# huangnengCSU/NanoSNP

Hardware: AMD Instinct MI355X
Metric: candidate SNP sites/sec (pileup encode + model fwd), 30x windows (higher is better)
Workload: dtype f32; 1 GPU; BASELINE configs[1]: pileup encode + PileupModel fwd, 1M synthetic 30x windows (G2) resident in HBM, batch=4096; batch=4096, windows_resident_per_gpu=1048576, streams=32, precision=fp32, parallelism=site-sharded x1, rooted gather of calls, world_size_observed=1, gather=torch

## Files before the change

### nanosnp_amd/csrc/nsnp_lstm_cell.hpp

```cpp
#pragma once

namespace nsnp_cell {

constexpr float LOG2E = 1.4426950408889634f;

static inline float lstm_gate_scale(int R) { return (R & 3) == 2 ? -2.0f * LOG2E : -LOG2E; }

__device__ __forceinline__ float cap64(float z) { return __builtin_amdgcn_fmed3f(z, -3.0e38f, 64.0f); }

__device__ __forceinline__ float lstm_cell(float zi, float zf, float zg, float zo, float c_prev, float& c_new)
{
    const float ei = __builtin_amdgcn_exp2f(zi);
    const float ef = __builtin_amdgcn_exp2f(zf);
    const float eo = __builtin_amdgcn_exp2f(zo);
    const float eg = __builtin_amdgcn_exp2f(cap64(zg));
    constexpr float K = -2.0f * LOG2E;
    const float tg = 1.0f + eg;
    const float ig = __builtin_fmaf(-K, eg, K) * __builtin_amdgcn_rcpf(__builtin_fmaf(ei, tg, tg));
    const float fg = __builtin_amdgcn_rcpf(1.0f + ef);
    const float cn = __builtin_fmaf(fg, c_prev, ig);
    const float ec = __builtin_amdgcn_exp2f(cap64(cn));
    c_new = cn;
    const float tc = 1.0f + ec;
    return (1.0f - ec) * __builtin_amdgcn_rcpf(__builtin_fmaf(eo, tc, tc));
}

struct CellSlices { float ei[4], ef[4], eo[4], eg[4], t[4], d[4], m[4], fg[4]; };
constexpr int CELL_SLICES = 80;

template <int I, typename Z4>
__device__ __forceinline__ void lstm_cell_slice(CellSlices& w, const Z4 (&z)[4], float (&c)[4], Z4& h)
{
    static_assert(I >= 0 && I < CELL_SLICES, "slice index");
    constexpr int st = I >> 2, u = I & 3;
    constexpr float K = -2.0f * LOG2E;
    if constexpr (st == 0) w.ei[u] = __builtin_amdgcn_exp2f(z[u][0]);
    else if constexpr (st == 1) w.ef[u] = __builtin_amdgcn_exp2f(z[u][1]);
    else if constexpr (st == 2) w.eo[u] = __builtin_amdgcn_exp2f(z[u][3]);
    else if constexpr (st == 3) w.t[u] = cap64(z[u][2]);
    else if constexpr (st == 4) w.eg[u] = __builtin_amdgcn_exp2f(w.t[u]);
    else if constexpr (st == 5) w.t[u] = 1.0f + w.eg[u];
    else if constexpr (st == 6) w.d[u] = __builtin_fmaf(w.ei[u], w.t[u], w.t[u]);
    else if constexpr (st == 7) w.d[u] = __builtin_amdgcn_rcpf(w.d[u]);
    else if constexpr (st == 8) w.m[u] = __builtin_fmaf(-K, w.eg[u], K);
    else if constexpr (st == 9) w.m[u] = w.m[u] * w.d[u];
    else if constexpr (st == 10) w.fg[u] = 1.0f + w.ef[u];
    else if constexpr (st == 11) w.fg[u] = __builtin_amdgcn_rcpf(w.fg[u]);
    else if constexpr (st == 12) c[u] = __builtin_fmaf(w.fg[u], c[u], w.m[u]);
    else if constexpr (st == 13) w.t[u] = cap64(c[u]);
    else if constexpr (st == 14) w.eg[u] = __builtin_amdgcn_exp2f(w.t[u]);
    else if constexpr (st == 15) w.t[u] = 1.0f + w.eg[u];
    else if constexpr (st == 16) w.d[u] = __builtin_fmaf(w.eo[u], w.t[u], w.t[u]);
    else if constexpr (st == 17) w.d[u] = __builtin_amdgcn_rcpf(w.d[u]);
    else if constexpr (st == 18) w.m[u] = 1.0f - w.eg[u];
    else h[u] = w.m[u] * w.d[u];
    if constexpr (st == 0) asm volatile("" : "+v"(w.ei[u]));
    else if constexpr (st == 1) asm volatile("" : "+v"(w.ef[u]));
    else if constexpr (st == 2) asm volatile("" : "+v"(w.eo[u]));
    else if constexpr (st == 4 || st == 14) asm volatile("" : "+v"(w.eg[u]));
    else if constexpr (st == 3 || st == 5 || st == 13 || st == 15) asm volatile("" : "+v"(w.t[u]));
    else if constexpr (st == 6 || st == 7 || st == 16 || st == 17) asm volatile("" : "+v"(w.d[u]));
    else if constexpr (st == 8 || st == 9 || st == 18) asm volatile("" : "+v"(w.m[u]));
    else if constexpr (st == 10 || st == 11) asm volatile("" : "+v"(w.fg[u]));
    else if constexpr (st == 12) asm volatile("" : "+v"(c[u]));
    else { float v = h[u]; asm volatile("" : "+v"(v)); h[u] = v; }
}

}
```

### nanosnp_amd/csrc/pileup_forward.hip

```cpp
#include "nsnp_common.hpp"
#include "nsnp_lstm_cell.hpp"
#include "nsnp_devclock.hpp"
#include "nsnp_bf16.hpp"
#include <type_traits>

namespace {

constexpr float LOG2E = 1.4426950408889634f;

__device__ __forceinline__ f32x4 mfma4(float a, float b, f32x4 c)
{
    return __builtin_amdgcn_mfma_f32_16x16x4f32(a, b, c, 0, 0, 0);
}
__device__ __forceinline__ float sigmoid_f(float x)
{
    return __builtin_amdgcn_rcpf(1.0f + __builtin_amdgcn_exp2f(-LOG2E * x));
}
__device__ __forceinline__ float tanh_f(float x)
{
    return __builtin_fmaf(-2.0f, __builtin_amdgcn_rcpf(1.0f + __builtin_amdgcn_exp2f((2.0f * LOG2E) * x)), 1.0f);
}

__device__ __forceinline__ float lstm_cell(float zi, float zf, float zg, float zo, float& c)
{
// ... 369 lines not shown
            Frag fr[2];
            f32x4 acc[2][4];
            load_b(0, fr[0]);
            gemm(fr[0], acc[0]);
#pragma unroll
            for (int sg = 0; sg < NSG; ++sg) {
                __builtin_amdgcn_sched_barrier(0);
                if (sg + 1 < NSG) load_b(sg + 1, fr[(sg + 1) & 1]);
                __builtin_amdgcn_sched_barrier(0);
                if (sg + 1 < NSG) gemm(fr[(sg + 1) & 1], acc[(sg + 1) & 1]);
                cell(sg, acc[sg & 1]);
                if (sg + 1 < NSG) {
#pragma unroll
                    for (int i = 0; i < 84; ++i) {
                        __builtin_amdgcn_sched_group_barrier(0x008, 1, 0);
                        __builtin_amdgcn_sched_group_barrier(0x400, 1, 0);
                        __builtin_amdgcn_sched_group_barrier(0x002, 1, 0);
                    }
                }
            }
            __builtin_amdgcn_sched_barrier(0);
        } else {
#pragma unroll
        for (int sg = 0; sg < NSG; ++sg) {
            const float* hr = &hx[cur ^ 1][16 * sg + n][4 * q];
            f32x4 hb0, hb1;
            if (s > 0) { hb0 = *reinterpret_cast<const f32x4*>(hr); hb1 = *reinterpret_cast<const f32x4*>(hr + 16); }
            const float* xr = &xx[cur][(16 * sg + n) * RS_XSROW];
            const f32x4 xb = *reinterpret_cast<const f32x4*>(xr + 4 * q);
            const float xl = xr[16 + q];
            f32x4 acc[4];
#pragma unroll
            for (int u = 0; u < 4; ++u) acc[u] = f32x4{0.f, 0.f, 0.f, 0.f};
            if (WXL) {
#pragma unroll
                for (int u = 0; u < 4; ++u) {
                    Wih[u] = *reinterpret_cast<const f32x4*>(&wxl[((wave * 4 + u) * 64 + lane) * 4]);
                    Wl[u] = wxl[4 * 4 * 64 * 4 + (wave * 4 + u) * 64 + lane];
                }
            }
#pragma unroll
            for (int e = 0; e < 4; ++e)
#pragma unroll
                for (int u = 0; u < 4; ++u) acc[u] = mfma4(Wih[u][e], xb[e], acc[u]);
#pragma unroll
            for (int u = 0; u < 4; ++u) acc[u] = mfma4(Wl[u], xl, acc[u]);
            if (s > 0) {
#define RS_KBLOCK(J, HB)                                                                               \
                _Pragma("unroll") for (int e = 0; e < 4; ++e)                                          \
                    _Pragma("unroll") for (int u = 0; u < 4; ++u) acc[u] = mfma4(Whh[u][J][e], HB[e], acc[u]);
                __builtin_amdgcn_sched_barrier(0);
                RS_KBLOCK(0, hb0)
                __builtin_amdgcn_sched_barrier(0);
                hb0 = *reinterpret_cast<const f32x4*>(hr + 32);
                RS_KBLOCK(1, hb1)
                __builtin_amdgcn_sched_barrier(0);
                hb1 = *reinterpret_cast<const f32x4*>(hr + 48);
                RS_KBLOCK(2, hb0)
                __builtin_amdgcn_sched_barrier(0);
                RS_KBLOCK(3, hb1)
#undef RS_KBLOCK
            }
            f32x4 hn;
#pragma unroll
            for (int u = 0; u < 4; ++u) {
                hn[u] = lstm_cell(acc[u][0], acc[u][1], acc[u][2], acc[u][3], c[sg][u]);
            }
            *reinterpret_cast<f32x4*>(&hx[cur][16 * sg + n][16 * wave + 4 * q]) = hn;
        }
        }
        if (s + 1 < PW) {
            stage_x(cur ^ 1);
            if (s + 2 < PW) load_x(dir ? t - 2 : t + 2);
        }
        lds_barrier();
    }
    flush_h((PW - 1) & 1, dir ? 0 : PW - 1);
    NSNP_DEVCLK_STOP(0)
}

constexpr int RX_PLANE = 4 * 16 * 8;
typedef float f32x2 __attribute__((ext_vector_type(2)));

__global__ __launch_bounds__(256, 3) void k_pileup_l0_rsx(
    const int32_t* __restrict__ x, const int64_t* __restrict__ center_idx, int64_t N,
    const float* __restrict__ whh0, const float* __restrict__ whh1,
    const __bf16* __restrict__ wx0, const __bf16* __restrict__ wx1,
    float* __restrict__ H0)
{
    __shared__ __attribute__((aligned(16))) float hx[2][16][RS_XROW];
    __shared__ __attribute__((aligned(16))) __bf16 xx[2][3][RX_PLANE];
    __shared__ __attribute__((aligned(16))) int xlvl[2][4];
    __shared__ int64_t xofs[9 * 16];
    const int dir = blockIdx.y;
    const int tid = threadIdx.x, lane = tid & 63, wave = __builtin_amdgcn_readfirstlane(tid >> 6);
    const int n = lane & 15, q = lane >> 4;
    NSNP_DEVCLK_START
    const int64_t base_site = (int64_t)blockIdx.x * 16;
    const int nrows = (int)min((int64_t)16, N - base_site);

    f32x4 Whh[4][4];
    b8 Wx[4][3];
    {
        const f32x4* __restrict__ ghh = reinterpret_cast<const f32x4*>(dir ? whh1 : whh0);
        const b8* __restrict__ gx = reinterpret_cast<const b8*>(dir ? wx1 : wx0);
#pragma unroll
        for (int u = 0; u < 4; ++u) {
#pragma unroll
            for (int j = 0; j < 4; ++j) Whh[u][j] = ghh[((4 * wave + u) * 4 + j) * 64 + lane];
#pragma unroll
            for (int p = 0; p < 3; ++p) Wx[u][p] = gx[((4 * wave + u) * 3 + p) * 64 + lane];
        }
    }

    const bool xon = tid < 9 * 16;
    const int xrow = min(wave < 2 ? lane >> 2 : n, nrows - 1);
    const int piece = wave < 2 ? 4 * wave + (lane & 3) : 8;
    const int xdst = wave < 2 ? 128 * wave + 2 * lane : 256 + 8 * n;
    const int32_t* const xwg = x + base_site * (PW * PC);
    unsigned xoff = (unsigned)(xrow * (PW * PC) + 2 * piece) * 4u;
    if (center_idx && xon) xofs[tid] = (center_idx[base_site + xrow] - PCENTER) * PC + 2 * piece;
    int2 xi = int2{0, 0};
    auto load_x = [&](int t) {
        if (!xon) return;
        if (center_idx) xi = *reinterpret_cast<const int2*>(x + xofs[tid] + t * PC);
        else {
            asm volatile("" : "+v"(xoff));
            xi = *reinterpret_cast<const int2*>(reinterpret_cast<const char*>(xwg + t * PC) + xoff);
        }
    };
    auto stage_x_split = [&](b2* d, int* lv) {
        __bf16 a0, a1, a2, c0, c1, c2;
        split3((float)xi.x, a0, a1, a2); split3((float)xi.y, c0, c1, c2);
        d[0] = b2{a0, c0}; d[RX_PLANE / 2] = b2{a1, c1}; d[RX_PLANE] = b2{a2, c2};
        const bool nz1 = (float)a1 != 0.f || (float)c1 != 0.f, nz2 = (float)a2 != 0.f || (float)c2 != 0.f;
        const int lvl = __ballot(nz2) != 0ull ? 2 : (__ballot(nz1) != 0ull ? 1 : 0);
        if (lane == 0) *lv = lvl;
    };
    auto stage_x = [&](int buf) {
        if (!xon) return;
        b2* const d = reinterpret_cast<b2*>(&xx[buf][0][xdst]);
        const bool big = (unsigned)xi.x + 256u > 512u || (unsigned)xi.y + 256u > 512u;
        if (__builtin_expect(__ballot(big) == 0ull, 1)) {
            d[0] = __builtin_convertvector(f32x2{(float)xi.x, (float)xi.y}, b2);
            d[RX_PLANE / 2] = b2{0, 0};
            d[RX_PLANE] = b2{0, 0};
            if (lane == 0) xlvl[buf][wave] = 0;
        } else {
            stage_x_split(d, &xlvl[buf][wave]);
        }
    };
    for (int i = tid; i < 2 * 3 * RX_PLANE / 8; i += 256) reinterpret_cast<b8*>(&xx[0][0][0])[i] = b8{0, 0, 0, 0, 0, 0, 0, 0};
    if (tid < 8) xlvl[tid >> 2][tid & 3] = 0;
    __syncthreads();
    if (tid < 32) xx[tid >> 4][0][2 * 128 + (tid & 15) * 8 + 2] = (__bf16)1.0f;
    load_x(dir ? PW - 1 : 0);
    stage_x(0);
    if (PW > 1) load_x(dir ? PW - 2 : 1);
    __syncthreads();

    float c[4];
#pragma unroll
    for (int u = 0; u < 4; ++u) c[u] = 0.f;

    float* const h0wg = H0 + (base_site * PW * 2 + dir) * 64;
    const int frow = tid >> 4, fcid = tid & 15;
    unsigned foff = (unsigned)(frow * (PW * 128) + 4 * fcid) * 4u;
    const float* const fl = &hx[0][frow][16 * (fcid & 3) + 4 * (fcid >> 2)];
    const bool fon = frow < nrows;
    auto flush_h = [&](int buf, int t) {
        asm volatile("" : "+v"(foff));
        if (fon)
            *reinterpret_cast<f32x4*>(reinterpret_cast<char*>(h0wg + t * 128) + foff) =
                *reinterpret_cast<const f32x4*>(fl + buf * (16 * RS_XROW));
    };

    for (int s = 0; s < PW; ++s) {
        const int t = dir ? PW - 1 - s : s;
        const int cur = s & 1;
        if (s > 0) flush_h(cur ^ 1, dir ? t + 1 : t - 1);
        const __bf16* xr = &xx[cur][0][q * 128 + n * 8];
        const b8 xb0 = *reinterpret_cast<const b8*>(xr);
        const i32x4 lv = *reinterpret_cast<const i32x4*>(xlvl[cur]);
        const int lvl = __builtin_amdgcn_readfirstlane(max(max(lv[0], lv[1]), max(lv[2], lv[3])));
        f32x4 hn;
        auto step = [&](auto lvl_tag) __attribute__((always_inline)) {
            constexpr int LVL = decltype(lvl_tag)::value;
            const float* hr = &hx[cur ^ 1][n][4 * q];
            f32x4 hb0, hb1;
            if (s > 0) { hb0 = *reinterpret_cast<const f32x4*>(hr); hb1 = *reinterpret_cast<const f32x4*>(hr + 16); }
            f32x4 acc[4];
#pragma unroll
            for (int u = 0; u < 4; ++u) acc[u] = f32x4{0.f, 0.f, 0.f, 0.f};
#pragma unroll
            for (int p = LVL; p >= 0; --p) {
                const b8 b = p ? *reinterpret_cast<const b8*>(xr + p * RX_PLANE) : xb0;
#pragma unroll
                for (int wp = 2; wp >= 0; --wp)
#pragma unroll
                    for (int u = 0; u < 4; ++u) acc[u] = __builtin_amdgcn_mfma_f32_16x16x32_bf16(Wx[u][wp], b, acc[u], 0, 0, 0);
            }
            if (s > 0) {
#define RS_KBLOCK(J, HB)                                                                               \
                _Pragma("unroll") for (int e = 0; e < 4; ++e)                                          \
                    _Pragma("unroll") for (int u = 0; u < 4; ++u) acc[u] = mfma4(Whh[u][J][e], HB[e], acc[u]);
                __builtin_amdgcn_sched_barrier(0);
                RS_KBLOCK(0, hb0)
                __builtin_amdgcn_sched_barrier(0);
                hb0 = *reinterpret_cast<const f32x4*>(hr + 32);
                RS_KBLOCK(1, hb1)
                __builtin_amdgcn_sched_barrier(0);
                hb1 = *reinterpret_cast<const f32x4*>(hr + 48);
                RS_KBLOCK(2, hb0)
                __builtin_amdgcn_sched_barrier(0);
                RS_KBLOCK(3, hb1)
#undef RS_KBLOCK
            }
#pragma unroll
            for (int u = 0; u < 4; ++u) hn[u] = lstm_cell(acc[u][0], acc[u][1], acc[u][2], acc[u][3], c[u]);
        };
        if (__builtin_expect(lvl == 0, 1)) step(std::integral_constant<int, 0>{});
        else if (lvl == 1)                 step(std::integral_constant<int, 1>{});
        else                               step(std::integral_constant<int, 2>{});
        *reinterpret_cast<f32x4*>(&hx[cur][n][16 * wave + 4 * q]) = hn;
        if (s + 1 < PW) {
            stage_x(cur ^ 1);
            if (s + 2 < PW) load_x(dir ? t - 2 : t + 2);
        }
        lds_barrier();
    }
    flush_h((PW - 1) & 1, dir ? 0 : PW - 1);
    NSNP_DEVCLK_STOP(0)
}

template <int... I, class F>
__device__ __forceinline__ void static_for_seq(std::integer_sequence<int, I...>, F&& f) { (f(std::integral_constant<int, I>{}), ...); }
template <int N, class F>
__device__ __forceinline__ void static_for(F&& f) { static_for_seq(std::make_integer_sequence<int, N>{}, f); }

constexpr bool rsxw_slice_is_trans(int i)
{
    const int st = i >> 2;
    return st == 0 || st == 1 || st == 2 || st == 4 || st == 7 || st == 11 || st == 14 || st == 17;
}
constexpr int rsxw_late_slice(int k) { return k < 8 ? 4 * (5 + (k & 1)) + (k >> 1) : 20 + k; }
constexpr int rsxw_mfmas_upto(int gap_t, int gap_v, int first, int nm, int last)
{
    int m = 0, run = 0;
    for (int k = first; k <= last; ++k) {
        const int quota = rsxw_slice_is_trans(rsxw_late_slice(k)) ? gap_t : gap_v;
        if (quota == 0) continue;
        if (m < nm && (m == 0 || run >= quota)) { ++m; run = 0; }
        ++run;
    }
    return m;
}

constexpr int RXP_IMAGE = PW * 3 * 16 * 8;
static_assert(3 * 16 * RS_XROW * 4 + 2 * 3 * RX_PLANE * 2 + 32 + RXP_IMAGE * 2 + 16 + 64 <= 160 * 1024 / 3, "three workgroups in a CU's 160 KB of LDS");

template <int GAP_T, int GAP_V, int GAP_FIRST, bool LATE_W0, bool PRESTAGE>
__device__ __forceinline__ void pileup_l0_rsxw_body(
    const int32_t* __restrict__ x, const int64_t* __restrict__ center_idx, int64_t N,
    const float* __restrict__ whh0, const float* __restrict__ whh1,
    const __bf16* __restrict__ wx0, const __bf16* __restrict__ wx1,
    float* __restrict__ H0)
{
    static_assert(GAP_T == 0 || GAP_V == 0, "one class of cell instruction paces the burst");
    static_assert(PW >= 3, "the pipeline stages three steps in its prologue");
    constexpr int LDS_ALIGN = PRESTAGE ? 64 : 16;
    __shared__ __attribute__((aligned(LDS_ALIGN))) float hx[3][16][RS_XROW];
    __shared__ __attribute__((aligned(LDS_ALIGN))) __bf16 xx[2][3][RX_PLANE];
    __shared__ __attribute__((aligned(LDS_ALIGN))) int xlvl[2][4];
    const int dir = blockIdx.y;
    const int tid = threadIdx.x, wave = __builtin_amdgcn_readfirstlane(tid >> 6);
    int lane = tid & 63, n = lane & 15, q = lane >> 4;
    NSNP_DEVCLK_START
    const int64_t base_site = (int64_t)blockIdx.x * 16;
    const int nrows = (int)min((int64_t)16, N - base_site);

    f32x4 Whh[4][4];
    b8 Wx[4][3];
    const f32x4* __restrict__ ghh = reinterpret_cast<const f32x4*>(dir ? whh1 : whh0);
    const b8* __restrict__ gx = reinterpret_cast<const b8*>(dir ? wx1 : wx0);
    if constexpr (!PRESTAGE) {
#pragma unroll
        for (int u = 0; u < 4; ++u) {
#pragma unroll
            for (int j = 0; j < 4; ++j) Whh[u][j] = ghh[((4 * wave + u) * 4 + j) * 64 + lane];
#pragma unroll
            for (int p = 0; p < 3; ++p) Wx[u][p] = gx[((4 * wave + u) * 3 + p) * 64 + lane];
        }
    }
    const bool xon = tid < 9 * 16;
    const int xrow = min(wave < 2 ? lane >> 2 : n, nrows - 1);
    const int piece = wave < 2 ? 4 * wave + (lane & 3) : 8;
    const int xdst = wave < 2 ? 128 * wave + 2 * lane : 256 + 8 * n;
    int frow = tid >> 4, fcid = tid & 15;
    float* fl = &hx[0][frow][16 * (fcid & 3) + 4 * (fcid >> 2)];
    int64_t* const xofs = reinterpret_cast<int64_t*>(fl + 2 * 16 * RS_XROW);
    int2 xi = int2{0, 0};
    auto tpos = [&](int u) { return dir ? PW - 1 - u : u; };

    const __bf16* ximg0 = nullptr, * ximg = nullptr;
    bool fast = false;
    if constexpr (PRESTAGE) {
        __shared__ __attribute__((aligned(16))) __bf16 img[RXP_IMAGE];
        __shared__ __attribute__((aligned(16))) int wbig[4];
        const int prow = min(frow, nrows - 1);
        const int2* const src = reinterpret_cast<const int2*>(
            x + (center_idx ? (center_idx[base_site + prow] - PCENTER) * PC : (base_site + prow) * (PW * PC)));
        constexpr int NP = (PW * 9 + 15) / 16;
        int2 wv[NP];
#pragma unroll
        for (int i = 0; i < NP; ++i) {
            const int p = fcid + 16 * i;
            wv[i] = (16 * i + 15 < PW * 9 || p < PW * 9) ? src[p] : int2{0, 0};
        }
        __builtin_amdgcn_sched_barrier(0);
#pragma unroll
        for (int u = 0; u < 4; ++u)
#pragma unroll
            for (int j = 0; j < 4; ++j) Whh[u][j] = ghh[((4 * wave + u) * 4 + j) * 64 + lane];
        __builtin_amdgcn_sched_barrier(0);
        bool big = false;
#pragma unroll
        for (int i = 0; i < NP; ++i) {
            const int p = fcid + 16 * i;
            if (16 * i + 15 < PW * 9 || p < PW * 9) {
                const int2 v = wv[i];
                const int pt = p / 9, pc = p - 9 * pt;
                big |= (unsigned)v.x + 256u > 512u || (unsigned)v.y + 256u > 512u;
                const b2 cv = __builtin_convertvector(f32x2{(float)v.x, (float)v.y}, b2);
                __bf16* const d = &img[(pt * 3 + (pc >> 2)) * 128 + frow * 8];
                if (pc < 8) *reinterpret_cast<b2*>(d + 2 * (pc & 3)) = cv;
                else        *reinterpret_cast<b8*>(d) = b8{cv[0], cv[1], (__bf16)1.0f, 0, 0, 0, 0, 0};
            }
        }
        const bool wave_big = __ballot(big) != 0ull;
        if (lane == 0) wbig[wave] = wave_big;
        __builtin_amdgcn_sched_barrier(0);
#pragma unroll
        for (int u = 0; u < 4; ++u)
#pragma unroll
            for (int p = 0; p < 3; ++p) Wx[u][p] = gx[((4 * wave + u) * 3 + p) * 64 + lane];
        lds_barrier();
        const i32x4 wb = *reinterpret_cast<const i32x4*>(wbig);
        fast = __builtin_amdgcn_readfirstlane(wb[0] | wb[1] | wb[2] | wb[3]) == 0;
        ximg0 = img;
    }
    bool qimg = q < 3;
    auto load_x = [&](int t) {
        if (!xon) return;
        xi = *reinterpret_cast<const int2*>(x + *xofs + t * PC);
    };
    auto stage_x_split = [&](b2* d, int* lv) {
        __bf16 a0, a1, a2, c0, c1, c2;
        split3((float)xi.x, a0, a1, a2); split3((float)xi.y, c0, c1, c2);
        d[0] = b2{a0, c0}; d[RX_PLANE / 2] = b2{a1, c1}; d[RX_PLANE] = b2{a2, c2};
        const bool nz1 = (float)a1 != 0.f || (float)c1 != 0.f, nz2 = (float)a2 != 0.f || (float)c2 != 0.f;
        const int lvl = __ballot(nz2) != 0ull ? 2 : (__ballot(nz1) != 0ull ? 1 : 0);
        if (lane == 0) *lv = lvl;
    };
    auto stage_x = [&](int buf) {
        if (!xon) return;
        b2* const d = reinterpret_cast<b2*>(&xx[buf][0][xdst]);
        const bool big = (unsigned)xi.x + 256u > 512u || (unsigned)xi.y + 256u > 512u;
        if (__builtin_expect(__ballot(big) == 0ull, 1)) {
            d[0] = __builtin_convertvector(f32x2{(float)xi.x, (float)xi.y}, b2);
            d[RX_PLANE / 2] = b2{0, 0};
            d[RX_PLANE] = b2{0, 0};
            if (lane == 0) xlvl[buf][wave] = 0;
        } else {
            stage_x_split(d, &xlvl[buf][wave]);
        }
    };
    auto stage_prologue = [&]() __attribute__((always_inline)) {
        if (xon) *xofs = (center_idx ? (center_idx[base_site + xrow] - PCENTER) * PC : (base_site + xrow) * (PW * PC)) + 2 * piece;
        for (int i = tid; i < 2 * 3 * RX_PLANE / 8; i += 256) reinterpret_cast<b8*>(&xx[0][0][0])[i] = b8{0, 0, 0, 0, 0, 0, 0, 0};
        if (tid < 8) xlvl[tid >> 2][tid & 3] = 0;
        __syncthreads();
        if (tid < 32) xx[tid >> 4][0][2 * 128 + (tid & 15) * 8 + 2] = (__bf16)1.0f;
        load_x(tpos(0)); stage_x(0);
        load_x(tpos(1)); stage_x(1);
        load_x(tpos(2));
        __syncthreads();
    };

    float c[4];
#pragma unroll
    for (int u = 0; u < 4; ++u) c[u] = 0.f;

    float* const h0wg = H0 + (base_site * PW * 2 + dir) * 64;
    unsigned foff = (unsigned)(frow * (PW * 128) + 4 * fcid) * 4u;
    bool fon = frow < nrows;
    auto flush_h = [&](int buf, int t) {
        asm volatile("" : "+v"(foff));
        if (fon)
            *reinterpret_cast<f32x4*>(reinterpret_cast<char*>(h0wg + t * 128) + foff) =
                *reinterpret_cast<const f32x4*>(fl + buf * (16 * RS_XROW));
    };

    constexpr int NM = LATE_W0 ? 8 : 12;
    auto read_x = [&](int buf, b8& xb0, int& lvl) __attribute__((always_inline)) {
        xb0 = *reinterpret_cast<const b8*>(&xx[buf][0][q * 128 + n * 8]);
        const i32x4 lv = *reinterpret_cast<const i32x4*>(xlvl[buf]);
        lvl = __builtin_amdgcn_readfirstlane(max(max(lv[0], lv[1]), max(lv[2], lv[3])));
    };
    auto project_block = [&](int buf, const b8& xb0, f32x4 (&acc)[4], auto lvl_tag) __attribute__((always_inline)) {
        constexpr int LVL = decltype(lvl_tag)::value;
        const __bf16* xr = &xx[buf][0][q * 128 + n * 8];
#pragma unroll
        for (int u = 0; u < 4; ++u) acc[u] = f32x4{0.f, 0.f, 0.f, 0.f};
#pragma unroll
        for (int p = LVL; p >= 0; --p) {
            const b8 b = p ? *reinterpret_cast<const b8*>(xr + p * RX_PLANE) : xb0;
#pragma unroll
            for (int wp = 2; wp >= (LATE_W0 && p == 0 ? 1 : 0); --wp)
#pragma unroll
                for (int u = 0; u < 4; ++u) {
                    acc[u] = __builtin_amdgcn_mfma_f32_16x16x32_bf16(Wx[u][wp], b, acc[u], 0, 0, 0);
                    __builtin_amdgcn_sched_barrier(0);
                }
        }
    };
    auto project_any = [&](int buf, const b8& xb0, int lvl, f32x4 (&acc)[4]) __attribute__((always_inline)) {
        if (__builtin_expect(lvl == 0, 1)) project_block(buf, xb0, acc, std::integral_constant<int, 0>{});
        else if (lvl == 1)                 project_block(buf, xb0, acc, std::integral_constant<int, 1>{});
        else                               project_block(buf, xb0, acc, std::integral_constant<int, 2>{});
    };

    auto read_image = [&](int t, b8& xb0) __attribute__((always_inline)) {
        if (qimg) xb0 = *reinterpret_cast<const b8*>(ximg + t * (3 * 128));
    };

    f32x4 acc[4];
    b8 xb;
    auto step = [&](int s, auto first_tag, auto last_tag, auto fast_tag) __attribute__((always_inline)) {
        constexpr bool FIRST = decltype(first_tag)::value, LAST = decltype(last_tag)::value, FAST = decltype(fast_tag)::value;
        const int t = tpos(s);
        const int cur = s & 1;
        const float* hr = &hx[cur ^ 1][n][4 * q];
        f32x4 hb0, hb1;
        if constexpr (!FIRST) { hb0 = *reinterpret_cast<const f32x4*>(hr); hb1 = *reinterpret_cast<const f32x4*>(hr + 16); }
        if constexpr (LATE_W0) {
            __builtin_amdgcn_sched_barrier(0);
#pragma unroll
            for (int u = 0; u < 4; ++u) acc[u] = __builtin_amdgcn_mfma_f32_16x16x32_bf16(Wx[u][0], xb, acc[u], 0, 0, 0);
            __builtin_amdgcn_sched_barrier(0);
        }
        int lvln = 0;
        if constexpr (FIRST) {
            if constexpr (FAST) read_image(tpos(s + 1), xb);
            else read_x(cur ^ 1, xb, lvln);
        } else {
#define RSXW_KBLOCK(J, HB)                                                                             \
            _Pragma("unroll") for (int e = 0; e < 4; ++e)                                              \
                _Pragma("unroll") for (int u = 0; u < 4; ++u) acc[u] = mfma4(Whh[u][J][e], HB[e], acc[u]);
            __builtin_amdgcn_sched_barrier(0);
            RSXW_KBLOCK(0, hb0)
            __builtin_amdgcn_sched_barrier(0);
            hb0 = *reinterpret_cast<const f32x4*>(hr + 32);
            RSXW_KBLOCK(1, hb1)
            __builtin_amdgcn_sched_barrier(0);
            hb1 = *reinterpret_cast<const f32x4*>(hr + 48);
            if constexpr (!LAST) {
                if constexpr (FAST) read_image(tpos(s + 1), xb);
                else read_x(cur ^ 1, xb, lvln);
            }
            RSXW_KBLOCK(2, hb0)
            __builtin_amdgcn_sched_barrier(0);
            flush_h(cur ^ 1, dir ? t + 1 : t - 1);
            RSXW_KBLOCK(3, hb1)
#undef RSXW_KBLOCK
        }
        __builtin_amdgcn_sched_barrier(0);
        nsnp_cell::CellSlices w;
        f32x4 hn;
        static_for<20>([&](auto ic) __attribute__((always_inline)) {
            constexpr int k = decltype(ic)::value, u = k / 5, st = k % 5 == 0 ? 3 : k % 5 == 4 ? 4 : k % 5 - 1;
            nsnp_cell::lstm_cell_slice<4 * st + u>(w, acc, c, hn);
        });
        __builtin_amdgcn_sched_barrier(0);
        auto burst = [&](auto from_tag, auto to_tag) __attribute__((always_inline)) {
            constexpr int FROM = decltype(from_tag)::value, TO = decltype(to_tag)::value;
            if constexpr (!LAST)
                static_for<TO - FROM>([&](auto mc) __attribute__((always_inline)) {
                    constexpr int m = FROM + decltype(mc)::value, u = m & 3, wp = 2 - (m >> 2);
                    if constexpr (m < 4) acc[u] = f32x4{0.f, 0.f, 0.f, 0.f};
                    acc[u] = __builtin_amdgcn_mfma_f32_16x16x32_bf16(Wx[u][wp], xb, acc[u], 0, 0, 0);
                    __builtin_amdgcn_sched_barrier(0);
                });
        };
        static_for<60>([&](auto kc) __attribute__((always_inline)) {
            constexpr int k = decltype(kc)::value;
            constexpr int before = rsxw_mfmas_upto(GAP_T, GAP_V, GAP_FIRST, NM, k - 1), upto = rsxw_mfmas_upto(GAP_T, GAP_V, GAP_FIRST, NM, k);
            burst(std::integral_constant<int, before>{}, std::integral_constant<int, upto>{});
            nsnp_cell::lstm_cell_slice<rsxw_late_slice(k)>(w, acc, c, hn);
            __builtin_amdgcn_sched_barrier(0);
        });
        *reinterpret_cast<f32x4*>(&hx[cur][n][16 * wave + 4 * q]) = hn;
        __builtin_amdgcn_sched_barrier(0);
        burst(std::integral_constant<int, rsxw_mfmas_upto(GAP_T, GAP_V, GAP_FIRST, NM, 59)>{}, std::integral_constant<int, NM>{});
        if constexpr (!LAST && !FAST) {
            if (__builtin_expect(lvln != 0, 0)) {
                if (lvln == 1) project_block(cur ^ 1, xb, acc, std::integral_constant<int, 1>{});
                else           project_block(cur ^ 1, xb, acc, std::integral_constant<int, 2>{});
            }
        }
        if constexpr (!LAST && !FAST) {
            stage_x(cur);
            load_x(tpos(s + 3 < PW ? s + 3 : PW - 1));
        }
        lds_barrier();
    };
    auto run = [&](auto fast_tag) __attribute__((always_inline)) {
        constexpr bool FAST = decltype(fast_tag)::value;
        if constexpr (FAST) {
            const int tid2 = 64 * wave + (int)__builtin_amdgcn_mbcnt_hi(~0u, __builtin_amdgcn_mbcnt_lo(~0u, 0u));
            lane = tid2 & 63; n = lane & 15; q = lane >> 4;
            frow = tid2 >> 4; fcid = tid2 & 15;
            fl = &hx[0][frow][16 * (fcid & 3) + 4 * (fcid >> 2)];
            foff = (unsigned)(frow * (PW * 128) + 4 * fcid) * 4u;
            fon = frow < nrows;
            qimg = q < 3;
            ximg = ximg0 + q * 128 + n * 8;
#pragma unroll
            for (int j = 0; j < 8; ++j) xb[j] = (__bf16)0.0f;
            read_image(tpos(0), xb);
            project_block(0, xb, acc, std::integral_constant<int, 0>{});
        } else {
            stage_prologue();
            int lvl0;
            read_x(0, xb, lvl0);
            project_any(0, xb, lvl0, acc);
            lds_barrier();
        }
        step(0, std::true_type{}, std::false_type{}, fast_tag);
        for (int s = 1; s < PW - 1; ++s) step(s, std::false_type{}, std::false_type{}, fast_tag);
        step(PW - 1, std::false_type{}, std::true_type{}, fast_tag);
        flush_h((PW - 1) & 1, dir ? 0 : PW - 1);
    };
    if constexpr (PRESTAGE) {
        if (__builtin_expect(fast, 1)) run(std::true_type{});
        else      run(std::false_type{});
    } else {
        run(std::false_type{});
    }
    NSNP_DEVCLK_STOP(0)
}

template <int GAP_T, int GAP_V, int GAP_FIRST, bool LATE_W0>
__global__ __launch_bounds__(256, 3) void k_pileup_l0_rsxw(
    const int32_t* __restrict__ x, const int64_t* __restrict__ center_idx, int64_t N,
    const float* __restrict__ whh0, const float* __restrict__ whh1,
    const __bf16* __restrict__ wx0, const __bf16* __restrict__ wx1,
    float* __restrict__ H0)
{
    pileup_l0_rsxw_body<GAP_T, GAP_V, GAP_FIRST, LATE_W0, false>(x, center_idx, N, whh0, whh1, wx0, wx1, H0);
}

template <int GAP_T, int GAP_V, int GAP_FIRST, bool LATE_W0>
__global__ __launch_bounds__(256, 3) void k_pileup_l0_rsxp(
    const int32_t* __restrict__ x, const int64_t* __restrict__ center_idx, int64_t N,
    const float* __restrict__ whh0, const float* __restrict__ whh1,
    const __bf16* __restrict__ wx0, const __bf16* __restrict__ wx1,
    float* __restrict__ H0)
{
    pileup_l0_rsxw_body<GAP_T, GAP_V, GAP_FIRST, LATE_W0, true>(x, center_idx, N, whh0, whh1, wx0, wx1, H0);
}
#ifndef RSXW_GAP_T
#define RSXW_GAP_T 1
#endif
#ifndef RSXW_GAP_V
#define RSXW_GAP_V 0
#endif
#ifndef RSXW_GAP_FIRST
#define RSXW_GAP_FIRST 24
#endif
#ifndef RSXW_LATE_W0
#define RSXW_LATE_W0 1
#endif

constexpr int rs32_l1_lds_bytes(int nsg) { return (2 * 16 * nsg * RS_H0ROW + 2 * 16 * nsg * RS_XROW) * 4; }

template <int NSG, bool STAGGER>
__global__ __launch_bounds__(512, 2) void k_pileup_l1_rs32(
    const float* __restrict__ H0, int64_t N,
    const float* __restrict__ wih0, const float* __restrict__ wih1,
    const float* __restrict__ whh0, const float* __restrict__ whh1,
    const float* __restrict__ bias0, const float* __restrict__ bias1,
    float* __restrict__ H1c)
{
    extern __shared__ f32x4 lds[];
    constexpr int NS = 16 * NSG;
    float* const h0s = reinterpret_cast<float*>(lds);
    float* const h1x = h0s + 2 * NS * RS_H0ROW;
    const int dir = blockIdx.y;
    const int tid = threadIdx.x, lane = tid & 63, wave = tid >> 6;
    const int n = lane & 15, q = lane >> 4;
    const int64_t base_site = (int64_t)blockIdx.x * NS;

    f32x4 Wih[2][8], Whh[2][4], bias[2];
    {
        const f32x4* __restrict__ gih = reinterpret_cast<const f32x4*>(dir ? wih1 : wih0);
        const f32x4* __restrict__ ghh = reinterpret_cast<const f32x4*>(dir ? whh1 : whh0);
        const f32x4* __restrict__ gb = reinterpret_cast<const f32x4*>(dir ? bias1 : bias0);
#pragma unroll
        for (int u = 0; u < 2; ++u) {
#pragma unroll
            for (int j = 0; j < 8; ++j) Wih[u][j] = gih[((2 * wave + u) * 8 + j) * 64 + lane];
#pragma unroll
            for (int j = 0; j < 4; ++j) Whh[u][j] = ghh[((2 * wave + u) * 4 + j) * 64 + lane];
            bias[u] = gb[(2 * wave + u) * 64 + lane];
        }
    }

    const int cid = tid & 31;
    const int slot = (cid & 16) + 4 * (cid & 3) + ((cid >> 2) & 3);
    f32x4 sreg[NSG];
    auto load_h0 = [&](int t) {
#pragma unroll
        for (int k = 0; k < NSG; ++k) {
            const int64_t site = base_site + (tid >> 5) + 16 * k;
            const int64_t sc = site < N ? site : N - 1;
            sreg[k] = *reinterpret_cast<const f32x4*>(H0 + (sc * PW + t) * 128 + 4 * cid);
        }
    };
    auto store_h0 = [&](int buf) {
#pragma unroll
        for (int k = 0; k < NSG; ++k)
            *reinterpret_cast<f32x4*>(h0s + ((size_t)buf * NS + (tid >> 5) + 16 * k) * RS_H0ROW + 4 * slot) = sreg[k];
    };
    auto tpos = [&](int u) { return dir ? PW - 1 - u : u; };
    load_h0(tpos(0)); store_h0(0);
    load_h0(tpos(1)); store_h0(1);
    __syncthreads();
    load_h0(tpos(2));

    f32x4 acc[NSG][2];
    auto input_part = [&](int sg, int buf, f32x4& a0, f32x4& a1) {
        const float* r0 = h0s + ((size_t)buf * NS + 16 * sg + n) * RS_H0ROW + 4 * q;
        a0 = bias[0]; a1 = bias[1];
#pragma unroll
        for (int j = 0; j < 8; ++j) {
            const f32x4 b4 = *reinterpret_cast<const f32x4*>(r0 + 64 * (j >> 2) + 16 * (j & 3));
#pragma unroll
            for (int e = 0; e < 4; ++e) {
                a0 = mfma4(Wih[0][j][e], b4[e], a0);
                a1 = mfma4(Wih[1][j][e], b4[e], a1);
            }
        }
    };
    const bool late = STAGGER && wave >= 4;
#pragma unroll
    for (int sg = 0; sg < NSG; ++sg) input_part(sg, 0, acc[sg][0], acc[sg][1]);
    lds_barrier();

    float c[NSG][2];
#pragma unroll
    for (int sg = 0; sg < NSG; ++sg) c[sg][0] = c[sg][1] = 0.f;

    for (int s = 0; s < PSTEPS1; ++s) {
        const int cur = s & 1;
        const float* hrb = h1x + (size_t)(cur ^ 1) * NS * RS_XROW;
        float* hwb = h1x + (size_t)cur * NS * RS_XROW;
#pragma unroll
        for (int sg = 0; sg < NSG; ++sg) {
            f32x4 nx0, nx1;
            if (late && s + 1 < PSTEPS1) input_part(sg, cur ^ 1, nx0, nx1);
            if (s > 0) {
                const float* r1 = hrb + (size_t)(16 * sg + n) * RS_XROW + 4 * q;
#pragma unroll
                for (int j = 0; j < 4; ++j) {
                    const f32x4 b4 = *reinterpret_cast<const f32x4*>(r1 + 16 * j);
#pragma unroll
                    for (int e = 0; e < 4; ++e) {
                        acc[sg][0] = mfma4(Whh[0][j][e], b4[e], acc[sg][0]);
                        acc[sg][1] = mfma4(Whh[1][j][e], b4[e], acc[sg][1]);
                    }
                }
            }
            float2 w2;
#pragma unroll
            for (int u = 0; u < 2; ++u) {
                const float h = lstm_cell(acc[sg][u][0], acc[sg][u][1], acc[sg][u][2], acc[sg][u][3], c[sg][u]);
                if (u == 0) w2.x = h; else w2.y = h;
            }
            *reinterpret_cast<float2*>(hwb + (size_t)(16 * sg + n) * RS_XROW + 16 * (wave >> 1) + 4 * q + 2 * (wave & 1)) = w2;
            if (s + 1 < PSTEPS1) {
                if (late) { acc[sg][0] = nx0; acc[sg][1] = nx1; }
                else input_part(sg, cur ^ 1, acc[sg][0], acc[sg][1]);
            }
        }
        if (s + 2 < PSTEPS1) {
            store_h0(cur);
            if (s + 3 < PSTEPS1) load_h0(tpos(s + 3));
        }
        lds_barrier();
    }
    const float* hfin = h1x + (size_t)((PSTEPS1 - 1) & 1) * NS * RS_XROW;
#pragma unroll
    for (int sg = 0; sg < NSG; ++sg) {
        const int64_t site = base_site + 16 * sg + n;
        if (site < N)
            *reinterpret_cast<float2*>(H1c + site * 128 + dir * 64 + q * 16 + 2 * wave) =
                *reinterpret_cast<const float2*>(hfin + (size_t)(16 * sg + n) * RS_XROW + 16 * (wave >> 1) + 4 * q + 2 * (wave & 1));
    }
}

constexpr int rs4_l1_lds_bytes(int nsg) { return (2 * 16 * nsg * RS_H0ROW + 2 * 16 * nsg * RS_XROW + 256) * 4; }

template <int NSG>
__global__ __launch_bounds__(256, 2) void k_pileup_l1_rs4(
    const float* __restrict__ H0, int64_t N,
    const float* __restrict__ wih0, const float* __restrict__ wih1,
    const float* __restrict__ whh0, const float* __restrict__ whh1,
    const float* __restrict__ bias0, const float* __restrict__ bias1,
    float* __restrict__ H1c)
{
    extern __shared__ f32x4 lds[];
    constexpr int NS = 16 * NSG;
    float* const h0s = reinterpret_cast<float*>(lds);
    float* const h1x = h0s + 2 * NS * RS_H0ROW;
    f32x4* const lbias = reinterpret_cast<f32x4*>(h1x + 2 * NS * RS_XROW);
    const int dir = blockIdx.y;
    const int tid = threadIdx.x, lane = tid & 63, wave = tid >> 6;
    const int n = lane & 15, q = lane >> 4;
    NSNP_DEVCLK_START
    const int64_t base_site = (int64_t)blockIdx.x * NS;

    f32x4 Wih[4][8], Whh[4][4];
    {
        const f32x4* __restrict__ gih = reinterpret_cast<const f32x4*>(dir ? wih1 : wih0);
        const f32x4* __restrict__ ghh = reinterpret_cast<const f32x4*>(dir ? whh1 : whh0);
#pragma unroll
        for (int u = 0; u < 4; ++u) {
#pragma unroll
            for (int j = 0; j < 8; ++j) Wih[u][j] = gih[((4 * wave + u) * 8 + j) * 64 + lane];
#pragma unroll
            for (int j = 0; j < 4; ++j) Whh[u][j] = ghh[((4 * wave + u) * 4 + j) * 64 + lane];
        }
        if (tid < 64) lbias[tid] = reinterpret_cast<const f32x4*>(dir ? bias1 : bias0)[(tid >> 2) * 64 + 16 * (tid & 3)];
    }

    const int cid = tid & 31;
    const int slot = (cid & 16) + 4 * (cid & 3) + ((cid >> 2) & 3);
    f32x4 sreg[2 * NSG];
    auto load_h0 = [&](int t) {
#pragma unroll
        for (int k = 0; k < 2 * NSG; ++k) {
            const int64_t site = base_site + (tid >> 5) + 8 * k;
            const int64_t sc = site < N ? site : N - 1;
            sreg[k] = *reinterpret_cast<const f32x4*>(H0 + (sc * PW + t) * 128 + 4 * cid);
        }
    };
    auto store_h0 = [&](int buf) {
#pragma unroll
        for (int k = 0; k < 2 * NSG; ++k)
            *reinterpret_cast<f32x4*>(h0s + ((size_t)buf * NS + (tid >> 5) + 8 * k) * RS_H0ROW + 4 * slot) = sreg[k];
    };
    load_h0(dir ? PW - 1 : 0);
    store_h0(0);
    if (PSTEPS1 > 1) load_h0(dir ? PW - 2 : 1);
    __syncthreads();

    float c[NSG][4];
#pragma unroll
    for (int sg = 0; sg < NSG; ++sg)
#pragma unroll
        for (int u = 0; u < 4; ++u) c[sg][u] = 0.f;

    for (int s = 0; s < PSTEPS1; ++s) {
        const int t = dir ? PW - 1 - s : s;
        const int cur = s & 1;
        const float* h0b = h0s + (size_t)cur * NS * RS_H0ROW;
        const float* hrb = h1x + (size_t)(cur ^ 1) * NS * RS_XROW;
        float* hwb = h1x + (size_t)cur * NS * RS_XROW;
#pragma unroll
        for (int sg = 0; sg < NSG; ++sg) {
            const float* r0 = h0b + (size_t)(16 * sg + n) * RS_H0ROW + 4 * q;
            f32x4 acc[4];
#pragma unroll
            for (int u = 0; u < 4; ++u) acc[u] = lbias[(4 * wave + u) * 4 + q];
#pragma unroll
            for (int j = 0; j < 8; ++j) {
                if (sg == 0 && j == 2 && s + 1 < PSTEPS1) {
                    __builtin_amdgcn_sched_barrier(0);
                    store_h0(cur ^ 1);
                    __builtin_amdgcn_sched_barrier(0);
                }
                if (sg == 0 && j == 5 && s + 2 < PSTEPS1) {
                    __builtin_amdgcn_sched_barrier(0);
                    load_h0(dir ? t - 2 : t + 2);
                    __builtin_amdgcn_sched_barrier(0);
                }
                const f32x4 b4 = *reinterpret_cast<const f32x4*>(r0 + 64 * (j >> 2) + 16 * (j & 3));
#pragma unroll
                for (int e = 0; e < 4; ++e)
#pragma unroll
                    for (int u = 0; u < 4; ++u) acc[u] = mfma4(Wih[u][j][e], b4[e], acc[u]);
            }
            if (s > 0) {
                const float* r1 = hrb + (size_t)(16 * sg + n) * RS_XROW + 4 * q;
#pragma unroll
                for (int j = 0; j < 4; ++j) {
                    const f32x4 b4 = *reinterpret_cast<const f32x4*>(r1 + 16 * j);
#pragma unroll
                    for (int e = 0; e < 4; ++e)
#pragma unroll
                        for (int u = 0; u < 4; ++u) acc[u] = mfma4(Whh[u][j][e], b4[e], acc[u]);
                }
            }
            f32x4 hn;
#pragma unroll
            for (int u = 0; u < 4; ++u) {
                hn[u] = lstm_cell(acc[u][0], acc[u][1], acc[u][2], acc[u][3], c[sg][u]);
            }
            *reinterpret_cast<f32x4*>(hwb + (size_t)(16 * sg + n) * RS_XROW + 16 * wave + 4 * q) = hn;
        }
        lds_barrier();
    }
    const float* hfin = h1x + (size_t)((PSTEPS1 - 1) & 1) * NS * RS_XROW;
#pragma unroll
    for (int sg = 0; sg < NSG; ++sg) {
        const int64_t site = base_site + 16 * sg + n;
        if (site < N)
            *reinterpret_cast<f32x4*>(H1c + site * 128 + dir * 64 + q * 16 + 4 * wave) =
                *reinterpret_cast<const f32x4*>(hfin + (size_t)(16 * sg + n) * RS_XROW + 16 * wave + 4 * q);
    }
    NSNP_DEVCLK_STOP(1)
}

constexpr int rs4w_l1_lds_bytes() { return rs4_l1_lds_bytes(1) + 4 * 4 * 2 * 64 * 16; }

template <int CELL_PER_GAP, int CELL_FIRST_GAP>
__global__ __launch_bounds__(256, 2) void k_pileup_l1_rs4w(
    const float* __restrict__ H0, int64_t N,
    const float* __restrict__ wih0, const float* __restrict__ wih1,
    const float* __restrict__ whh0, const float* __restrict__ whh1,
    const float* __restrict__ bias0, const float* __restrict__ bias1,
    float* __restrict__ H1c)
{
// ... 756 lines not shown
```

Baseline: 21.40 million sites/s.

## Restructure prestage image writes, unroll fast-path steps by parity, in-place cell FMA

The prestage loader now has each lane fetch one channel pair across all positions with a fixed stride. It writes those pairs and the constant-one padding to the bf16 LDS image directly, and uses a float max for the overflow check instead of the per-element divide-and-branch loop. The fast recurrence loop is unrolled in pairs so the double-buffer parity is a compile-time constant. The image read advances a byte offset incrementally rather than recomputing the address. The LSTM cell-state update is emitted as an in-place v_fma to avoid an extra register move. Together these aim to cut address arithmetic, register pressure and instruction count in the hot step loop, at the cost of more code size and a static assumption that PC==18 and PW is an odd number in [32,48].

```diff
diff --git a/nanosnp_amd/csrc/nsnp_lstm_cell.hpp b/nanosnp_amd/csrc/nsnp_lstm_cell.hpp
--- a/nanosnp_amd/csrc/nsnp_lstm_cell.hpp
+++ b/nanosnp_amd/csrc/nsnp_lstm_cell.hpp
@@ -28,7 +28,7 @@
 struct CellSlices { float ei[4], ef[4], eo[4], eg[4], t[4], d[4], m[4], fg[4]; };
 constexpr int CELL_SLICES = 80;
 
-template <int I, typename Z4>
+template <int I, bool C_IN_PLACE = false, typename Z4>
 __device__ __forceinline__ void lstm_cell_slice(CellSlices& w, const Z4 (&z)[4], float (&c)[4], Z4& h)
 {
     static_assert(I >= 0 && I < CELL_SLICES, "slice index");
@@ -46,6 +46,7 @@
     else if constexpr (st == 9) w.m[u] = w.m[u] * w.d[u];
     else if constexpr (st == 10) w.fg[u] = 1.0f + w.ef[u];
     else if constexpr (st == 11) w.fg[u] = __builtin_amdgcn_rcpf(w.fg[u]);
+    else if constexpr (st == 12 && C_IN_PLACE) asm volatile("v_fma_f32 %0, %1, %0, %2" : "+v"(c[u]) : "v"(w.fg[u]), "v"(w.m[u]));
     else if constexpr (st == 12) c[u] = __builtin_fmaf(w.fg[u], c[u], w.m[u]);
     else if constexpr (st == 13) w.t[u] = cap64(c[u]);
     else if constexpr (st == 14) w.eg[u] = __builtin_amdgcn_exp2f(w.t[u]);
@@ -62,7 +63,7 @@
     else if constexpr (st == 6 || st == 7 || st == 16 || st == 17) asm volatile("" : "+v"(w.d[u]));
     else if constexpr (st == 8 || st == 9 || st == 18) asm volatile("" : "+v"(w.m[u]));
     else if constexpr (st == 10 || st == 11) asm volatile("" : "+v"(w.fg[u]));
-    else if constexpr (st == 12) asm volatile("" : "+v"(c[u]));
+    else if constexpr (st == 12) { if constexpr (!C_IN_PLACE) asm volatile("" : "+v"(c[u])); }
     else { float v = h[u]; asm volatile("" : "+v"(v)); h[u] = v; }
 }
 
diff --git a/nanosnp_amd/csrc/pileup_forward.hip b/nanosnp_amd/csrc/pileup_forward.hip
--- a/nanosnp_amd/csrc/pileup_forward.hip
+++ b/nanosnp_amd/csrc/pileup_forward.hip
@@ -695,48 +695,59 @@
     int2 xi = int2{0, 0};
     auto tpos = [&](int u) { return dir ? PW - 1 - u : u; };
 
-    const __bf16* ximg0 = nullptr, * ximg = nullptr;
+    const __bf16* ximg0 = nullptr;
+    int ximg = 0;
     bool fast = false;
     if constexpr (PRESTAGE) {
         __shared__ __attribute__((aligned(16))) __bf16 img[RXP_IMAGE];
         __shared__ __attribute__((aligned(16))) int wbig[4];
+        static_assert(PC == 18 && PW >= 32 && PW <= 48, "nine channel pairs a position; a row's 16 lanes write the constants of positions k, k + 16, k + 32");
         const int prow = min(frow, nrows - 1);
+        const int pcp = min(fcid, 8);
         const int2* const src = reinterpret_cast<const int2*>(
-            x + (center_idx ? (center_idx[base_site + prow] - PCENTER) * PC : (base_site + prow) * (PW * PC)));
-        constexpr int NP = (PW * 9 + 15) / 16;
-        int2 wv[NP];
-#pragma unroll
-        for (int i = 0; i < NP; ++i) {
-            const int p = fcid + 16 * i;
-            wv[i] = (16 * i + 15 < PW * 9 || p < PW * 9) ? src[p] : int2{0, 0};
-        }
+            x + (center_idx ? (center_idx[base_site + prow] - PCENTER) * PC : (base_site + prow) * (PW * PC))) + pcp;
+        int2 wv[PW];
+#pragma unroll
+        for (int i = 0; i < PW; ++i) wv[i] = src[(PC / 2) * i];
         __builtin_amdgcn_sched_barrier(0);
 #pragma unroll
         for (int u = 0; u < 4; ++u)
 #pragma unroll
             for (int j = 0; j < 4; ++j) Whh[u][j] = ghh[((4 * wave + u) * 4 + j) * 64 + lane];
         __builtin_amdgcn_sched_barrier(0);
-        bool big = false;
-#pragma unroll
-        for (int i = 0; i < NP; ++i) {
-            const int p = fcid + 16 * i;
-            if (16 * i + 15 < PW * 9 || p < PW * 9) {
-                const int2 v = wv[i];
-                const int pt = p / 9, pc = p - 9 * pt;
-                big |= (unsigned)v.x + 256u > 512u || (unsigned)v.y + 256u > 512u;
-                const b2 cv = __builtin_convertvector(f32x2{(float)v.x, (float)v.y}, b2);
-                __bf16* const d = &img[(pt * 3 + (pc >> 2)) * 128 + frow * 8];
-                if (pc < 8) *reinterpret_cast<b2*>(d + 2 * (pc & 3)) = cv;
-                else        *reinterpret_cast<b8*>(d) = b8{cv[0], cv[1], (__bf16)1.0f, 0, 0, 0, 0, 0};
-            }
-        }
-        const bool wave_big = __ballot(big) != 0ull;
+        float cmax = 0.f;
+        unsigned cv[PW];
+#pragma unroll
+        for (int i = 0; i < PW; ++i) {
+            const float a = (float)wv[i].x, b = (float)wv[i].y;
+            cmax = __builtin_fmaxf(__builtin_fmaxf(__builtin_fabsf(a), __builtin_fabsf(b)), cmax);
+            cv[i] = __builtin_bit_cast(unsigned, __builtin_convertvector(f32x2{a, b}, b2));
+            asm volatile("" : "+v"(cv[i]), "+v"(cmax));
+        }
+        char* const imgb = reinterpret_cast<char*>(img);
+        if (fcid < 9) {
+            char* const d = imgb + (pcp >> 2) * 256 + frow * 16 + (pcp & 3) * 4;
+#pragma unroll
+            for (int i = 0; i < PW; ++i) *reinterpret_cast<unsigned*>(d + i * (3 * 256)) = cv[i];
+        }
+        {
+            char* const d = imgb + fcid * (3 * 256) + 2 * 256 + frow * 16 + 4;
+            auto ones = [&](int i) __attribute__((always_inline)) {
+                *reinterpret_cast<unsigned*>(d + i * (3 * 256)) = 0x3F80u;
+                *reinterpret_cast<uint2*>(d + i * (3 * 256) + 4) = uint2{0u, 0u};
+            };
+            ones(0);
+            ones(16);
+            if (fcid < PW - 32) ones(32);
+        }
+        const bool wave_big = __ballot(cmax > 256.0f) != 0ull;
         if (lane == 0) wbig[wave] = wave_big;
         __builtin_amdgcn_sched_barrier(0);
+        const b8* const gxl = gx + 4 * wave * 3 * 64 + lane;
 #pragma unroll
         for (int u = 0; u < 4; ++u)
 #pragma unroll
-            for (int p = 0; p < 3; ++p) Wx[u][p] = gx[((4 * wave + u) * 3 + p) * 64 + lane];
+            for (int p = 0; p < 3; ++p) Wx[u][p] = gxl[(u * 3 + p) * 64];
         lds_barrier();
         const i32x4 wb = *reinterpret_cast<const i32x4*>(wbig);
         fast = __builtin_amdgcn_readfirstlane(wb[0] | wb[1] | wb[2] | wb[3]) == 0;
@@ -823,16 +834,20 @@
         else                               project_block(buf, xb0, acc, std::integral_constant<int, 2>{});
     };
 
-    auto read_image = [&](int t, b8& xb0) __attribute__((always_inline)) {
-        if (qimg) xb0 = *reinterpret_cast<const b8*>(ximg + t * (3 * 128));
+    const int ximg_step = dir ? -3 * 256 : 3 * 256;
+    auto read_image_next = [&](b8& xb0) __attribute__((always_inline)) {
+        ximg += ximg_step;
+        asm volatile("" : "+v"(ximg));
+        if (qimg) xb0 = *reinterpret_cast<const b8*>(reinterpret_cast<const char*>(ximg0) + ximg);
     };
 
     f32x4 acc[4];
     b8 xb;
-    auto step = [&](int s, auto first_tag, auto last_tag, auto fast_tag) __attribute__((always_inline)) {
+    auto step = [&](int s, auto first_tag, auto last_tag, auto fast_tag, auto par_tag) __attribute__((always_inline)) {
         constexpr bool FIRST = decltype(first_tag)::value, LAST = decltype(last_tag)::value, FAST = decltype(fast_tag)::value;
+        constexpr int PAR = decltype(par_tag)::value;
         const int t = tpos(s);
-        const int cur = s & 1;
+        const int cur = PAR >= 0 ? PAR : (s & 1);
         const float* hr = &hx[cur ^ 1][n][4 * q];
         f32x4 hb0, hb1;
         if constexpr (!FIRST) { hb0 = *reinterpret_cast<const f32x4*>(hr); hb1 = *reinterpret_cast<const f32x4*>(hr + 16); }
@@ -844,7 +859,7 @@
         }
         int lvln = 0;
         if constexpr (FIRST) {
-            if constexpr (FAST) read_image(tpos(s + 1), xb);
+            if constexpr (FAST) read_image_next(xb);
             else read_x(cur ^ 1, xb, lvln);
         } else {
 #define RSXW_KBLOCK(J, HB)                                                                             \
@@ -858,7 +873,7 @@
             __builtin_amdgcn_sched_barrier(0);
             hb1 = *reinterpret_cast<const f32x4*>(hr + 48);
             if constexpr (!LAST) {
-                if constexpr (FAST) read_image(tpos(s + 1), xb);
+                if constexpr (FAST) read_image_next(xb);
                 else read_x(cur ^ 1, xb, lvln);
             }
             RSXW_KBLOCK(2, hb0)
@@ -872,7 +887,7 @@
         f32x4 hn;
         static_for<20>([&](auto ic) __attribute__((always_inline)) {
             constexpr int k = decltype(ic)::value, u = k / 5, st = k % 5 == 0 ? 3 : k % 5 == 4 ? 4 : k % 5 - 1;
-            nsnp_cell::lstm_cell_slice<4 * st + u>(w, acc, c, hn);
+            nsnp_cell::lstm_cell_slice<4 * st + u, true>(w, acc, c, hn);
         });
         __builtin_amdgcn_sched_barrier(0);
         auto burst = [&](auto from_tag, auto to_tag) __attribute__((always_inline)) {
@@ -889,7 +904,7 @@
             constexpr int k = decltype(kc)::value;
             constexpr int before = rsxw_mfmas_upto(GAP_T, GAP_V, GAP_FIRST, NM, k - 1), upto = rsxw_mfmas_upto(GAP_T, GAP_V, GAP_FIRST, NM, k);
             burst(std::integral_constant<int, before>{}, std::integral_constant<int, upto>{});
-            nsnp_cell::lstm_cell_slice<rsxw_late_slice(k)>(w, acc, c, hn);
+            nsnp_cell::lstm_cell_slice<rsxw_late_slice(k), true>(w, acc, c, hn);
             __builtin_amdgcn_sched_barrier(0);
         });
         *reinterpret_cast<f32x4*>(&hx[cur][n][16 * wave + 4 * q]) = hn;
@@ -917,10 +932,10 @@
             foff = (unsigned)(frow * (PW * 128) + 4 * fcid) * 4u;
             fon = frow < nrows;
             qimg = q < 3;
-            ximg = ximg0 + q * 128 + n * 8;
+            ximg = q * 256 + n * 16 + tpos(0) * (3 * 256);
 #pragma unroll
             for (int j = 0; j < 8; ++j) xb[j] = (__bf16)0.0f;
-            read_image(tpos(0), xb);
+            if (qimg) xb = *reinterpret_cast<const b8*>(reinterpret_cast<const char*>(ximg0) + ximg);
             project_block(0, xb, acc, std::integral_constant<int, 0>{});
         } else {
             stage_prologue();
@@ -929,9 +944,23 @@
             project_any(0, xb, lvl0, acc);
             lds_barrier();
         }
-        step(0, std::true_type{}, std::false_type{}, fast_tag);
-        for (int s = 1; s < PW - 1; ++s) step(s, std::false_type{}, std::false_type{}, fast_tag);
-        step(PW - 1, std::false_type{}, std::true_type{}, fast_tag);
+        using par_any = std::integral_constant<int, -1>;
+        using par_even = std::integral_constant<int, 0>;
+        using par_odd = std::integral_constant<int, 1>;
+        if constexpr (FAST) {
+            static_assert(PW % 2 == 1, "steps 1 .. PW - 3 in pairs, then an odd and the last, even, one");
+            step(0, std::true_type{}, std::false_type{}, fast_tag, par_even{});
+            for (int s = 1; s < PW - 2; s += 2) {
+                step(s, std::false_type{}, std::false_type{}, fast_tag, par_odd{});
+                step(s + 1, std::false_type{}, std::false_type{}, fast_tag, par_even{});
+            }
+            step(PW - 2, std::false_type{}, std::false_type{}, fast_tag, par_odd{});
+            step(PW - 1, std::false_type{}, std::true_type{}, fast_tag, par_even{});
+        } else {
+            step(0, std::true_type{}, std::false_type{}, fast_tag, par_any{});
+            for (int s = 1; s < PW - 1; ++s) step(s, std::false_type{}, std::false_type{}, fast_tag, par_any{});
+            step(PW - 1, std::false_type{}, std::true_type{}, fast_tag, par_any{});
+        }
         flush_h((PW - 1) & 1, dir ? 0 : PW - 1);
     };
     if constexpr (PRESTAGE) {
```

Result: no change. 21.52 million sites/s, median of 6 (+0.6%).
